# gasparian/CRNN-OCR-lite

Measured on AMD Instinct MI355X. Metric: text-line images/sec (train step), higher is better.
Workload: dtype bf16; 1 GPU; BASELINE configs[1]: 100x32x1 text lines, batch 256/GPU, max_len 23, time_dense_size 128, n_units 256 BiLSTM, STN on, dropout on, CTC, Adam(1e-4,b1=.5,clipnorm 5), bf16 MFMA products, bf16 conv-stack tensors in HBM, fp32 accumulate/statistics/RNN/optimizer (outside the 1e-3 parity tolerance: see parity_mode for the fp32 step); global_batch=256, parallelism=dp1, parity_mode_backward_planes=2 (16 significant bits per factor; CRNN_FLAG_THREE_PLANE_BACKWARD = strict)

## Files before the change

### crnn-ocr-lite_amd/crnn_mi355x/native.py

```python
import ctypes
import os
import re
import subprocess

HERE = os.path.dirname(os.path.abspath(__file__))
PKG_ROOT = os.path.dirname(HERE)
REPO_ROOT = os.path.dirname(PKG_ROOT)
HEADER = os.path.join(REPO_ROOT, "include", "crnn_mi355x.h")
CSRC = os.path.join(PKG_ROOT, "csrc")
LIB_PATH = os.path.join(PKG_ROOT, "libcrnn_mi355x.so")
HOOKS_HEADER = os.path.join(REPO_ROOT, "include", "crnn_testhooks.h")
HOOKS_PATH = os.path.join(PKG_ROOT, "libcrnn_testhooks.so")
SOURCES = ["gemm.hip", "gemm_nt.hip", "gemm_wres.hip", "gemm_wres3.hip", "gemm_wgrad.hip", "gemm_wgrad3.hip", "gemm_pres.hip", "conv.hip", "conv_bwd_fused.hip", "dwconv_stream.hip", "dwconv_bwd_stream.hip", "stn.hip", "rnn.hip", "rnn_persist.hip", "gru_persist.hip", "ctc.hip", "dense.hip", "beam.hip", "score.hip", "optim.hip", "ingest.hip", "model.hip"]


class crnn_config(ctypes.Structure):
    _fields_ = [(n, ctypes.c_int) for n in
                ("batch", "imgh", "imgw", "num_classes", "max_len", "tds", "units", "gru", "stn", "dropout", "mfma_bf16", "flags")]


FLAG_RNN_STEP_KERNELS = 1
FLAG_GEMM_TILE_KERNELS = 2
FLAG_NO_DW_BN_FUSION = 8
FLAG_NO_DW_BWD_FUSION = 16
FLAG_DW_TILE_KERNEL = 32
FLAG_RNN_LINEAR_CLUSTERS = 64
FLAG_NO_BN_STATS_FUSION = 128
FLAG_F32_MFMA_GEMMS = 256
FLAG_BN2_DW_FUSION = 1024
FLAG_BN2_STATS_FUSION = 2048
FLAG_BLOCK1_KERNELS = 16384
FLAG_LOC_NET_KERNELS = 8192
FLAG_THREE_PLANE_BACKWARD = 65536
FLAG_TWO_PLANE_FORWARD = 131072
FLAG_NO_GRADIENT_PLANES = 262144
FLAG_NO_POOL_ARGMAX_Q = 524288
FLAG_NO_BN2_DW_FUSION = 4096
RNN_XCD_LOCAL = 0x100


_CTYPE = [("crnn_stream_t", ctypes.c_void_p), ("size_t", ctypes.c_size_t), ("uint64_t", ctypes.c_uint64),
          ("uint32_t", ctypes.c_uint32), ("long", ctypes.c_long), ("int", ctypes.c_int), ("float", ctypes.c_float),
          ("double", ctypes.c_double)]


def _ctype_of(decl):
    decl = decl.strip()
    if "*" in decl:
        return ctypes.c_void_p
    for key, ct in _CTYPE:
        if re.search(r"\b%s\b" % key, decl):
            return ct
    raise ValueError("cannot map C type: %r" % decl)


def parse_header(path=HEADER):
    src = open(path).read()
    src = re.sub(r"/\*.*?\*/", " ", src, flags=re.S)
    src = re.sub(r"typedef\s+struct\s*\{.*?\}\s*\w+\s*;", " ", src, flags=re.S)
# ... 83 lines not shown
```

### crnn-ocr-lite_amd/csrc/conv.hip

```cpp
#include "common.h"
#include <stdlib.h>

#define BN_EPS 1e-3f
#ifndef DW_NT
#define DW_NT 256
#endif

template <int VEC>
struct VecF { float v[VEC]; };

#ifndef CRNN_NT_BN_BWD2
#define CRNN_NT_BN_BWD2 1
#endif
#ifndef CRNN_NT_BN_ACT
#define CRNN_NT_BN_ACT 1
#endif
template <int VEC, typename T>
__device__ __forceinline__ VecF<VEC> vload_nt(const T* p);
template <int VEC, bool NT, typename T>
__device__ __forceinline__ VecF<VEC> vload_s(const T* p);
template <int VEC, typename T>
__device__ __forceinline__ VecF<VEC> vload(const T* p) {
  VecF<VEC> r;
  if (VEC == 8) {
// ... 1508 lines not shown
    for (int r = rt; r < 128 && r0 + r < M; r += RT) {
      const float av = relu6f(fmaf(d[r0 + r], sc, sh));
      VecF<8> o;
#pragma unroll
      for (int e = 0; e < 8; ++e) o.v[e] = av * wv[e];
      vstore<8>(&q[(r0 + r) * N + 8 * cg], o);
#pragma unroll
      for (int e = 0; e < 8; ++e) {
        float v = o.v[e];
        if (sizeof(T) == 2) v = __uint_as_float(pack2_bf16(v, 0.f) << 16);
        s[e] += v; ss[e] = fmaf(v, v, ss[e]);
      }
    }
#pragma unroll
  for (int e = 0; e < 8; ++e) { red[0][tid * 8 + e] = s[e]; red[1][tid * 8 + e] = ss[e]; }
  __syncthreads();
  if (tid < 2 * N) {
    const int v = tid / N, c = tid % N;
    float acc = 0.f;
    for (int r = 0; r < RT; ++r) acc += red[v][(r * CG + c / 8) * 8 + (c & 7)];
    stats[((long)blockIdx.x * 2 + v) * N + c] = acc;
  }
}
template <typename T>
__global__ __launch_bounds__(256) void pw1_bn_bwd_kernel(const float* __restrict__ d, const float* __restrict__ bn1, const float* __restrict__ w,
                                                         const T* __restrict__ dq, float* __restrict__ da, float* __restrict__ partials,
                                                         float* __restrict__ bnparts, long M, int N, int rows_per_chunk) {
  __shared__ float red[256 * 8];
  __shared__ float sred[2][256];
  const int CG = N / 8, RT = 256 / CG, tid = threadIdx.x, cg = tid % CG, rt = tid / CG;
  const long r0 = (long)blockIdx.x * rows_per_chunk;
  long r1 = r0 + rows_per_chunk; if (r1 > M) r1 = M;
  const float mu = bn1[0], inv = 1.0f / sqrtf(bn1[1] + BN_EPS), sc = bn1[2], sh = bn1[3];
  VecF<8> wl = vload<8>(w + 8 * cg);
  float s[8], sg = 0.f, sq = 0.f;
#pragma unroll
  for (int e = 0; e < 8; ++e) s[e] = 0.f;
  if (rt < RT)
    for (long r = r0 + rt; r < r1; r += RT) {
      const float dv = d[r], t = fmaf(dv, sc, sh), av = relu6f(t);
      VecF<8> g = vload<8>(&dq[r * N + 8 * cg]);
      float acc = 0.f;
#pragma unroll
      for (int e = 0; e < 8; ++e) { s[e] = fmaf(av, g.v[e], s[e]); acc = fmaf(g.v[e], wl.v[e], acc); }
      for (int o = 1; o < CG; o <<= 1) acc += __shfl_xor(acc, o, 64);
      if (cg == 0) {
        da[r] = acc;
        const float gy = (t > 0.f && t < 6.f) ? acc : 0.f;
        sg += gy; sq = fmaf(gy, (dv - mu) * inv, sq);
      }
    }
#pragma unroll
  for (int e = 0; e < 8; ++e) red[tid * 8 + e] = s[e];
  sred[0][tid] = sg; sred[1][tid] = sq;
  __syncthreads();
  if (tid < N) {
    float acc = 0.f;
    for (int r = 0; r < RT; ++r) acc += red[(r * CG + tid / 8) * 8 + (tid & 7)];
    partials[(long)blockIdx.x * N + tid] = acc;
  }
  if (tid < 2) {
    float acc = 0.f;
    for (int r = 0; r < RT; ++r) acc += sred[tid][r * CG];
    bnparts[(long)blockIdx.x * 2 + tid] = acc;
// ... 141 lines not shown
  if (!pw1_ok(N, q) || M <= 0) return CRNN_ERR_UNSUPPORTED;
  const int blocks = cdiv(M, 128);
  if (dt_q == CRNN_BF16) hipLaunchKernelGGL(pw1_bn_fwd_kernel<bf16_t>, dim3(blocks), dim3(256), 0, stream, d, in_bnstate, w, (bf16_t*)q, stat_partials, M, N);
  else hipLaunchKernelGGL(pw1_bn_fwd_kernel<float>, dim3(blocks), dim3(256), 0, stream, d, in_bnstate, w, (float*)q, stat_partials, M, N);
  CRNN_LAUNCH_CHECK();
  return CRNN_OK;
}
extern "C" int crnn_dwconv_c1_bwd_rows(int B, int H, int W) { return cdiv((long)B * H * W, 1024); }
extern "C" int crnn_dwconv3x3_c1_bwd(const float* d, const float* da, const float* bnstate, const float* coef, const float* x, const float* k, float* dx, float* dk,
                                     float* scratch, int B, int H, int W, hipStream_t stream) {
  if (!d || !da || !bnstate || !coef || !x || !k || !dk || !scratch || B <= 0 || H <= 0 || W <= 0) return CRNN_ERR_ARG;
  if ((long)B * H * W >= (1L << 31) || W > C1B_MAXW) return CRNN_ERR_UNSUPPORTED;
  const int rows = crnn_dwconv_c1_bwd_rows(B, H, W);
  hipLaunchKernelGGL(dwconv_c1_bwd_kernel, dim3(rows), dim3(256), 0, stream, d, da, bnstate, coef, x, k, dx, scratch, B, H, W);
  CRNN_LAUNCH_CHECK();
  return crnn_partials_sum(scratch, rows, 9, dk, 1.f, stream);
}
extern "C" int crnn_pw1_bn_bwd_rows(long M) { return cdiv(M, colreduce_rpc(M)); }
extern "C" int crnn_pw1_bn_bwd(const float* d, const float* in_bnstate, const float* w, const void* dq, float* da, float* dw, float* scratch,
                               float* bn_stat_partials, long M, int N, int dt_q, hipStream_t stream) {
  if (!d || !in_bnstate || !w || !dq || !da || !dw || !scratch || !bn_stat_partials) return CRNN_ERR_ARG;
  if (!pw1_ok(N, dq) || M <= 0 || N < 8) return CRNN_ERR_UNSUPPORTED;
  const int rpc = colreduce_rpc(M), chunks = cdiv(M, rpc);
  if (dt_q == CRNN_BF16) hipLaunchKernelGGL(pw1_bn_bwd_kernel<bf16_t>, dim3(chunks), dim3(256), 0, stream, d, in_bnstate, w, (const bf16_t*)dq, da, scratch, bn_stat_partials, M, N, rpc);
  else hipLaunchKernelGGL(pw1_bn_bwd_kernel<float>, dim3(chunks), dim3(256), 0, stream, d, in_bnstate, w, (const float*)dq, da, scratch, bn_stat_partials, M, N, rpc);
  CRNN_LAUNCH_CHECK();
  return crnn_partials_sum(scratch, chunks, N, dw, 1.f, stream);
}
```

### crnn-ocr-lite_amd/csrc/model.hip

```cpp
#include "common.h"
#include "crnn_mi355x.h"
#include <string.h>
#include <stdio.h>
#include <string>
#include <vector>

namespace {

struct BlockSpec { int cout, ph, pw; };
const BlockSpec kBlocks[7] = {{64, 1, 1}, {128, 1, 1}, {256, 2, 2}, {256, 1, 1}, {512, 1, 2}, {512, 1, 1}, {512, 1, 1}};
bool pool_argmax_q(const crnn_config* cfg, int block) {
  const int ph = kBlocks[block - 1].ph, pw = kBlocks[block - 1].pw;
  return !(cfg->flags & CRNN_FLAG_NO_POOL_ARGMAX_Q) && ((ph == 2 && pw == 2) || (ph == 1 && pw == 2));
}
const float kDropBlock = 0.1f, kDropDense1 = 0.4f, kDropRnn = 0.2f;
const uint32_t kLayerDense1 = 8, kLayerRnn = 9;

struct Tensor { std::string name; long off; long size; int ndim; int dims[4]; int dtype = CRNN_F32; };

struct Dims {
  int B, H0, W0, Hp, Wp, T, feat, C, L, tds, u, G, stn_flat;
  int Hs1, Ws1, Ho1, Wo1, Hs2, Ws2, Ho2, Wo2;
  int bh[8], bw[8], bc[8];
};
// ... 939 lines not shown
  Ctx ca = c; if (aux) { ca.s = aux; ca.side = true; }
  float* gA = c.w("gA"); float* gB = c.w("gB"); float* gC = c.w("gC");
  hipEvent_t gB_free = nullptr, gC_free = nullptr;
  int bn2_stats_rows = 0;
  for (int i = 7; i >= 1; --i) {
    std::string p = std::to_string(i), bp = "b" + p;
    const int H = d.bh[i], W = d.bw[i], ci = d.bc[i - 1], co = d.bc[i];
    const long M = (long)B * H * W;
    const int dtd = c.dt("d" + p), dtq = c.dt("q" + p);
    const bool fused_bf = i > 1 && dtd == CRNN_BF16 && c.dt("x" + std::to_string(i - 1)) == CRNN_BF16 && !(cfg->flags & CRNN_FLAG_NO_DW_BWD_FUSION) &&
                          crnn_dwconv_bwd_fused_supported(H, W, ci) == CRNN_OK;
    const bool fused_f32 = i > 1 && dtd == CRNN_F32 && dtq == CRNN_F32 && c.dt("x" + std::to_string(i - 1)) == CRNN_F32 &&
                           !(cfg->flags & (CRNN_FLAG_NO_DW_BWD_FUSION | CRNN_FLAG_DW_TILE_KERNEL)) &&
                           crnn_dwconv_bwd_stream_supported_ex(B, H, W, ci, CRNN_F32) == CRNN_OK &&
                           aligned16(c.w("d" + p), c.w("x" + std::to_string(i - 1)), c.p(bp + "_dw"), c.w("coef")) && aligned16(gA, gB, gC, c.w("bn1s" + p));
    const bool fused_dw = fused_bf || fused_f32;
    int bn1_stats_rows = 0;
    const bool dq_planes = !fused_bf && pw_products(cfg) == 2 && conv_planes(cfg, true) == 2 && dtq == CRNN_F32 && dtd == CRNN_F32 && fuse_dw_bn_x3(cfg, dtd, dtq, ci) &&
                           !(cfg->flags & (CRNN_FLAG_GEMM_TILE_KERNELS | CRNN_FLAG_NO_BN_STATS_FUSION | CRNN_FLAG_NO_GRADIENT_PLANES)) &&
                           (kBlocks[i - 1].ph * kBlocks[i - 1].pw == 1 || crnn_knob("CRNN_DQPL_POOL", 1)) &&
                           crnn_gemm_pres_supported(M, ci, co, 2) == CRNN_OK && crnn_pwconv_wgrad_planes_stream_supported(M, co, ci) == CRNN_OK &&
                           crnn_pwconv_wgrad_planes_stream_scratch_bytes(M, co, ci) <= kGemmScratchBytes &&
                           aligned16(c.w("d" + p), c.w("q" + p), c.w("bn1s" + p), c.p(bp + "_pw")) && aligned16(gA, gB, gC, c.w("partials"));
    CRNN_TRY(fj.wait(gB_free)); gB_free = nullptr;
    if (bn2_stats_rows > 0) {
      CRNN_TRY(crnn_bn_bwd_finalize(c.w("bn2parts"), bn2_stats_rows, co, M, c.g(bp + "_bn2_g"), c.g(bp + "_bn2_b"), c.w("coef"), stream));
      if (dq_planes)
        CRNN_TRY(crnn_bn_bwd_apply_planes_ex(c.w("q" + p), gA, c.w("bn2s" + p), c.w("coef"), gB, M * co, 2, B, H, W, co, kBlocks[i - 1].ph, kBlocks[i - 1].pw,
                                             cfg->dropout ? kDropBlock : 0.f, seed, (uint32_t)i, stream));
      else
      CRNN_TRY(crnn_bn_bwd_apply_ex(c.w("q" + p), gA, c.w("bn2s" + p), c.w("coef"), gB, B, H, W, co, kBlocks[i - 1].ph, kBlocks[i - 1].pw,
                                    cfg->dropout ? kDropBlock : 0.f, seed, (uint32_t)i, dtq, stream));
      bn2_stats_rows = 0;
    } else if (use_qmax(c, i))
      CRNN_TRY(crnn_bn_bwd_qmax_ex(c.w("q" + p), c.w("qm" + p), gA, c.w("bn2s" + p), c.p(bp + "_bn2_g"), dq_planes ? nullptr : gB, dq_planes ? gB : nullptr, M * co,
                                   dq_planes ? 2 : 0, c.g(bp + "_bn2_g"), c.g(bp + "_bn2_b"), c.w("partials"), c.w("coef"), B, H, W, co, kBlocks[i - 1].ph,
                                   kBlocks[i - 1].pw, cfg->dropout ? kDropBlock : 0.f, seed, (uint32_t)i, dtq, stream));
    else if (dq_planes)
      CRNN_TRY(crnn_bn_bwd_planes_ex(c.w("q" + p), gA, c.w("bn2s" + p), c.p(bp + "_bn2_g"), gB, M * co, 2, c.g(bp + "_bn2_g"), c.g(bp + "_bn2_b"), c.w("partials"),
                                     c.w("coef"), B, H, W, co, kBlocks[i - 1].ph, kBlocks[i - 1].pw, cfg->dropout ? kDropBlock : 0.f, seed, (uint32_t)i, stream));
    else
    CRNN_TRY(crnn_bn_bwd_ex(c.w("q" + p), gA, c.w("bn2s" + p), c.p(bp + "_bn2_g"), gB, c.g(bp + "_bn2_g"), c.g(bp + "_bn2_b"), c.w("partials"),
                            c.w("coef"), B, H, W, co, kBlocks[i - 1].ph, kBlocks[i - 1].pw, cfg->dropout ? kDropBlock : 0.f, seed, (uint32_t)i, dtq, stream));
    if (block1_fused(cfg, ci, dtd)) {
      const int rows = crnn_pw1_bn_bwd_rows(M);
      float* bnp = c.w("partials");
      CRNN_TRY(crnn_pw1_bn_bwd(c.w("d" + p), c.w("bn1s" + p), c.p(bp + "_pw"), gB, gA, c.g(bp + "_pw"), bnp + ((2L * rows + 63) & ~63L), bnp, M, co, dtq, stream));
      bn1_stats_rows = rows;
    } else if (ci == 1 && dtd == CRNN_F32) {
      CRNN_TRY(crnn_pw1_bwd(c.w("a" + p), c.p(bp + "_pw"), gB, gA, c.g(bp + "_pw"), c.w("partials"), M, co, dtq, stream));
    } else {
      const bool side = fj.on && fused_dw;
      const Ctx& cw = side ? ca : c;
      if (side) CRNN_TRY(fj.fork());
      if (fuse_dw_bn(cfg, dtd, dtq, ci)) {
        int rc = CRNN_ERR_UNSUPPORTED;
        if (!(cfg->flags & CRNN_FLAG_GEMM_TILE_KERNELS) && crnn_pwconv_wgrad_stream_supported(M, co, ci) == CRNN_OK)
          rc = crnn_pwconv_bnrelu6_wgrad_stream(c.w("d" + p), c.w("bn1s" + p), gB, c.g(bp + "_pw"), M, co, ci, cw.scratch(), kGemmScratchBytes, cw.s);
        if (rc == CRNN_ERR_UNSUPPORTED)
          rc = crnn_pwconv_bnrelu6_wgrad(c.w("d" + p), c.w("bn1s" + p), gB, c.g(bp + "_pw"), M, co, ci, cw.scratch(), kGemmScratchBytes, cw.s);
        CRNN_TRY(rc);
      }
      else if (fuse_dw_bn_x3(cfg, dtd, dtq, ci) && aligned16(c.w("d" + p), c.w("q" + p), c.w("bn1s" + p), c.p(bp + "_pw"))) {
        int rc = CRNN_ERR_UNSUPPORTED;
        if (dq_planes) { CRNN_TRY(crnn_pwconv_bnrelu6_wgrad_planes_stream_gp(c.w("d" + p), c.w("bn1s" + p), gB, M * co, c.g(bp + "_pw"), M, co, ci, cw.scratch(), kGemmScratchBytes, cw.s)); rc = CRNN_OK; }
        if (rc == CRNN_ERR_UNSUPPORTED)
          rc = (conv_planes(cfg, true) == 2 ? crnn_pwconv_bnrelu6_wgrad_f32x2 : crnn_pwconv_bnrelu6_wgrad_f32x3)(
              c.w("d" + p), c.w("bn1s" + p), gB, c.g(bp + "_pw"), M, co, ci, cw.scratch(), kGemmScratchBytes, cw.s);
        CRNN_TRY(rc);
      }
      else CRNN_TRY(gemm_t(cw, 2, c.w("a" + p), dtd, gB, dtq, c.g(bp + "_pw"), CRNN_F32, ci, co, (int)M, ci, co, co, nullptr, 0, 0, 0, conv_planes(cfg, true)));
// ... 148 lines not shown
```

### include/crnn_mi355x.h

```cpp
#ifndef CRNN_MI355X_H
#define CRNN_MI355X_H
#include <stddef.h>
#include <stdint.h>
#ifdef __cplusplus
extern "C" {
#endif

typedef struct ihipStream_t* crnn_stream_t;

typedef struct {
  int batch;
  int imgh, imgw;
  int num_classes;
  int max_len;
  int tds;
  int units;
  int gru;
  int stn;
  int dropout;
  int mfma_bf16;
  int flags;
} crnn_config;
#define CRNN_FLAG_BLOCK1_KERNELS 16384
#define CRNN_FLAG_LOC_NET_KERNELS 8192
#define CRNN_FLAG_NO_BN2_DW_FUSION 4096
#define CRNN_FLAG_BN2_STATS_FUSION 2048
#define CRNN_FLAG_BN2_DW_FUSION 1024
#define CRNN_FLAG_DW_TILE_KERNEL 32
#define CRNN_FLAG_NO_DW_BWD_FUSION 16
#define CRNN_FLAG_NO_DW_BN_FUSION 8
#define CRNN_FLAG_GEMM_TILE_KERNELS 2
#define CRNN_FLAG_THREE_PLANE_BACKWARD 65536
#define CRNN_FLAG_TWO_PLANE_FORWARD 131072
#define CRNN_FLAG_NO_GRADIENT_PLANES 262144
#define CRNN_FLAG_NO_POOL_ARGMAX_Q 524288
#define CRNN_FLAG_F32_MFMA_GEMMS 256
#define CRNN_FLAG_NO_BN_STATS_FUSION 128
#define CRNN_FLAG_RNN_LINEAR_CLUSTERS 64
#define CRNN_FLAG_RNN_STEP_KERNELS 1

int  crnn_num_params(const crnn_config* cfg);
long crnn_params_total(const crnn_config* cfg);
int  crnn_param_info(const crnn_config* cfg, int idx, char* name, int name_cap, long* offset, long* size,
                     int* ndim, int* dims );
int  crnn_bn_total(const crnn_config* cfg);
int  crnn_bn_info(const crnn_config* cfg, int idx, char* name, int name_cap, int* offset, int* channels, long* count);
int  crnn_time_steps(const crnn_config* cfg);

size_t crnn_workspace_bytes(const crnn_config* cfg);
int  crnn_ws_tensor(const crnn_config* cfg, const char* name, long* offset, long* count);
int  crnn_block_output_fused(const crnn_config* cfg, int block);
int  crnn_ws_tensor_info(const crnn_config* cfg, const char* name, long* offset, long* count, int* dtype);


int crnn_forward(const crnn_config* cfg, const float* params, const float* bn_mean, const float* bn_var,
                 const float* x, float* ws, size_t ws_bytes, float* y_pred, int train, uint64_t seed,
                 crnn_stream_t stream);
int crnn_forward_ex(const crnn_config* cfg, const float* params, const float* bn_mean, const float* bn_var,
// ... 85 lines not shown
int crnn_pwconv_bnrelu6_wgrad_planes_stream_gp(const float* d, const float* in_bnstate, const void* g_planes, long g_plane_stride, float* dw, long M, int N, int K,
                                               float* scratch, size_t scratch_bytes, crnn_stream_t stream);
int crnn_gemm_tn_planes_stream(const float* A, int lda, const float* B, int ldb, float* C, int ldc, int M, int N, long K, float* scratch,
                               size_t scratch_bytes, crnn_stream_t stream);
int crnn_gemm_nt_f32x2_stream(const float* A0, const float* W0, const float* A1, const float* W1, float* Y, int M, int N, int K, int lda, int ldw, int ldy,
                              crnn_stream_t stream);
int crnn_gemm_pres_supported(long M, int N, int K, int planes);
int crnn_gemm_pres_stat_rows(long M, int N, int K, int planes);
int crnn_gemm_pres_bnstats(const void* dq_planes, long plane_stride, const float* w, float* da, long M, int N, int K, int planes, const float* d,
                           const float* bnstate, float* stat_partials, void* a_planes, long a_stride, int a_count, crnn_stream_t stream);
int crnn_pw1_fwd(const float* a, const float* w, void* q, long M, int N, float* stat_partials, int dt_q, crnn_stream_t stream);
int crnn_pw1_fwd_folded(const float* a, const float* w, void* y, long M, int N, const float* out_bnstate, int dt_y, crnn_stream_t stream);
int crnn_pw1_bwd(const float* a, const float* w, const void* dq, float* da, float* dw, float* scratch, long M, int N, int dt_q,
                 crnn_stream_t stream);
int crnn_dwconv_c1_stat_rows(int B, int H, int W);
int crnn_dwconv3x3_c1_fwd(const float* x, const float* k, float* out, float* stat_partials, int B, int H, int W, crnn_stream_t stream);
int crnn_pw1_bn_fwd(const float* d, const float* in_bnstate, const float* w, void* q, long M, int N, float* stat_partials, int dt_q, crnn_stream_t stream);
int crnn_dwconv_c1_bwd_rows(int B, int H, int W);
int crnn_dwconv3x3_c1_bwd(const float* d, const float* da, const float* bnstate, const float* coef, const float* x, const float* k, float* dx, float* dk,
                          float* scratch, int B, int H, int W, crnn_stream_t stream);
int crnn_pw1_bn_bwd_rows(long M);
int crnn_pw1_bn_bwd(const float* d, const float* in_bnstate, const float* w, const void* dq, float* da, float* dw, float* scratch, float* bn_stat_partials,
                    long M, int N, int dt_q, crnn_stream_t stream);
int crnn_dwconv3x3_bn_relu6_fwd(const void* x, const float* k, const float* bnstate, void* out, int B, int H, int W, int C,
                                int dtype, crnn_stream_t stream);
int crnn_dwconv_fwd_stream_supported(int B, int H, int W, int C);
int crnn_dwconv_fwd_stream_rows(int B, int H, int W, int C);
int crnn_dwconv3x3_fwd_stream(const void* x, const float* k, void* out, float* stat_partials, const float* bnstate, int B, int H, int W, int C,
                              int flip, crnn_stream_t stream);
int crnn_dwconv3x3_fwd_stream_ex(const void* x, const float* k, void* out, float* stat_partials, const float* bnstate, int B, int H, int W, int C,
                                 int flip, int out_order, crnn_stream_t stream);
int crnn_dwconv_fwd_stream_pro_supported(int B, int H, int W, int C);
int crnn_dwconv3x3_fwd_stream_pro(const void* q, const float* pro_bnstate, float rate, const void* keep, const float* k, void* out,
                                  float* stat_partials, int B, int H, int W, int C, crnn_stream_t stream);
int crnn_transpose_batch(const float* src, void* dst, int n, const long* in_off, const long* out_off, const int* R, const int* C,
                         int dt_out, crnn_stream_t stream);
int crnn_dwconv3x3_fwd_ex(const void* x, const float* k, void* out, float* stat_partials, int B, int H, int W, int C, int flip,
                          int dtype, crnn_stream_t stream);
int crnn_dwconv3x3_wgrad_ex(const void* x, const void* g, float* dk, float* scratch, int B, int H, int W, int C, int dtype,
                            crnn_stream_t stream);
int crnn_colreduce_ex(const void* x, float* partials, long M, int C, int ld, int nv, int dtype, crnn_stream_t stream);
int crnn_bn_act_pool_drop_ex(const void* x, const float* bnstate, void* y, int B, int H, int W, int C, int ph, int pw, float rate,
                             uint64_t seed, uint32_t layer, int dt_in, int dt_out, crnn_stream_t stream);
int crnn_bn_bwd_ex(const void* x, const void* g, const float* bnstate, const float* gamma, void* dx, float* dgamma, float* dbeta,
                   float* scratch_partials, float* coef, int B, int H, int W, int C, int ph, int pw, float rate, uint64_t seed,
                   uint32_t layer, int dtype, crnn_stream_t stream);
// ... 213 lines not shown
```

Baseline: 43560 images/sec.

## Fuse BN2 backward apply into pointwise-conv backward kernels to skip dq materialization

Adds a fused pointwise-conv backward kernel (MFMA bf16) that recomputes the BN2/ReLU6/dropout backward input gradient on the fly from q and g. It also computes the BN1-relu6 activation from d and produces both da and the weight gradient in one pass. A variant of the block-1 pw1 backward kernel applies the BN backward inline the same way. This removes the separate bn_bwd apply pass and the HBM round trip of the dq tensor for unpooled blocks. It adds a large, complex kernel with split-K partial reductions and more launch conditions.

```diff
diff --git a/crnn-ocr-lite_amd/crnn_mi355x/native.py b/crnn-ocr-lite_amd/crnn_mi355x/native.py
--- a/crnn-ocr-lite_amd/crnn_mi355x/native.py
+++ b/crnn-ocr-lite_amd/crnn_mi355x/native.py
@@ -11,7 +11,7 @@
 LIB_PATH = os.path.join(PKG_ROOT, "libcrnn_mi355x.so")
 HOOKS_HEADER = os.path.join(REPO_ROOT, "include", "crnn_testhooks.h")
 HOOKS_PATH = os.path.join(PKG_ROOT, "libcrnn_testhooks.so")
-SOURCES = ["gemm.hip", "gemm_nt.hip", "gemm_wres.hip", "gemm_wres3.hip", "gemm_wgrad.hip", "gemm_wgrad3.hip", "gemm_pres.hip", "conv.hip", "conv_bwd_fused.hip", "dwconv_stream.hip", "dwconv_bwd_stream.hip", "stn.hip", "rnn.hip", "rnn_persist.hip", "gru_persist.hip", "ctc.hip", "dense.hip", "beam.hip", "score.hip", "optim.hip", "ingest.hip", "model.hip"]
+SOURCES = ["gemm.hip", "gemm_nt.hip", "gemm_wres.hip", "gemm_wres3.hip", "gemm_wgrad.hip", "gemm_wgrad3.hip", "gemm_pres.hip", "gemm_pwbwd.hip", "conv.hip", "conv_bwd_fused.hip", "dwconv_stream.hip", "dwconv_bwd_stream.hip", "stn.hip", "rnn.hip", "rnn_persist.hip", "gru_persist.hip", "ctc.hip", "dense.hip", "beam.hip", "score.hip", "optim.hip", "ingest.hip", "model.hip"]
 
 
 class crnn_config(ctypes.Structure):
@@ -35,6 +35,7 @@
 FLAG_TWO_PLANE_FORWARD = 131072
 FLAG_NO_GRADIENT_PLANES = 262144
 FLAG_NO_POOL_ARGMAX_Q = 524288
+FLAG_NO_PW_BWD_FUSION = 1048576
 FLAG_NO_BN2_DW_FUSION = 4096
 RNN_XCD_LOCAL = 0x100
 
diff --git a/crnn-ocr-lite_amd/csrc/conv.hip b/crnn-ocr-lite_amd/csrc/conv.hip
--- a/crnn-ocr-lite_amd/csrc/conv.hip
+++ b/crnn-ocr-lite_amd/csrc/conv.hip
@@ -1554,10 +1554,11 @@
     stats[((long)blockIdx.x * 2 + v) * N + c] = acc;
   }
 }
-template <typename T>
+template <typename T, bool APPLY = false>
 __global__ __launch_bounds__(256) void pw1_bn_bwd_kernel(const float* __restrict__ d, const float* __restrict__ bn1, const float* __restrict__ w,
                                                          const T* __restrict__ dq, float* __restrict__ da, float* __restrict__ partials,
-                                                         float* __restrict__ bnparts, long M, int N, int rows_per_chunk) {
+                                                         float* __restrict__ bnparts, long M, int N, int rows_per_chunk, BnBwdArgsT<T> ap,
+                                                         const float* __restrict__ coef) {
   __shared__ float red[256 * 8];
   __shared__ float sred[2][256];
   const int CG = N / 8, RT = 256 / CG, tid = threadIdx.x, cg = tid % CG, rt = tid / CG;
@@ -1568,10 +1569,36 @@
   float s[8], sg = 0.f, sq = 0.f;
 #pragma unroll
   for (int e = 0; e < 8; ++e) s[e] = 0.f;
+  VecF<8> sc2, sh2, Pc, Qc;
+  float inv_keep = 1.f;
+  if constexpr (APPLY) {
+    const int c0 = 8 * cg;
+    const VecF<8> mu2 = vload<8>(ap.bnstate + c0), var2 = vload<8>(ap.bnstate + N + c0);
+    sc2 = vload<8>(ap.bnstate + 2 * N + c0); sh2 = vload<8>(ap.bnstate + 3 * N + c0);
+    const VecF<8> c1 = vload<8>(coef + c0), c2 = vload<8>(coef + N + c0);
+#pragma unroll
+    for (int e = 0; e < 8; ++e) bn_bwd_pq(sc2.v[e], c1.v[e], c2.v[e], mu2.v[e], 1.0f / sqrtf(var2.v[e] + BN_EPS), Pc.v[e], Qc.v[e]);
+    inv_keep = ap.rate > 0.f ? 1.f / (1.f - ap.rate) : 1.f;
+  }
   if (rt < RT)
     for (long r = r0 + rt; r < r1; r += RT) {
       const float dv = d[r], t = fmaf(dv, sc, sh), av = relu6f(t);
-      VecF<8> g = vload<8>(&dq[r * N + 8 * cg]);
+      VecF<8> g;
+      if constexpr (APPLY) {
+        const VecF<8> xv = vload<8>(&ap.x[r * N + 8 * cg]);
+        const VecF<8> gy = bn_gy_vec<8, false, T>(ap, r, 8 * cg, xv, sc2, sh2, inv_keep);
+#pragma unroll
+        for (int e = 0; e < 8; ++e) g.v[e] = bn_bwd_dx_pq(xv.v[e], gy.v[e], sc2.v[e], Pc.v[e], Qc.v[e]);
+        if constexpr (sizeof(T) == 2) {
+#pragma unroll
+          for (int e = 0; e < 8; e += 2) {
+            const unsigned pk = pack2_bf16(g.v[e], g.v[e + 1]);
+            g.v[e] = __uint_as_float(pk << 16); g.v[e + 1] = __uint_as_float(pk & 0xffff0000u);
+          }
+        }
+      } else {
+        g = vload<8>(&dq[r * N + 8 * cg]);
+      }
       float acc = 0.f;
 #pragma unroll
       for (int e = 0; e < 8; ++e) { s[e] = fmaf(av, g.v[e], s[e]); acc = fmaf(g.v[e], wl.v[e], acc); }
@@ -1759,8 +1786,29 @@
   if (!d || !in_bnstate || !w || !dq || !da || !dw || !scratch || !bn_stat_partials) return CRNN_ERR_ARG;
   if (!pw1_ok(N, dq) || M <= 0 || N < 8) return CRNN_ERR_UNSUPPORTED;
   const int rpc = colreduce_rpc(M), chunks = cdiv(M, rpc);
-  if (dt_q == CRNN_BF16) hipLaunchKernelGGL(pw1_bn_bwd_kernel<bf16_t>, dim3(chunks), dim3(256), 0, stream, d, in_bnstate, w, (const bf16_t*)dq, da, scratch, bn_stat_partials, M, N, rpc);
-  else hipLaunchKernelGGL(pw1_bn_bwd_kernel<float>, dim3(chunks), dim3(256), 0, stream, d, in_bnstate, w, (const float*)dq, da, scratch, bn_stat_partials, M, N, rpc);
+  if (dt_q == CRNN_BF16) hipLaunchKernelGGL(pw1_bn_bwd_kernel<bf16_t>, dim3(chunks), dim3(256), 0, stream, d, in_bnstate, w, (const bf16_t*)dq, da, scratch, bn_stat_partials, M, N, rpc, BnBwdArgsT<bf16_t>{}, nullptr);
+  else hipLaunchKernelGGL(pw1_bn_bwd_kernel<float>, dim3(chunks), dim3(256), 0, stream, d, in_bnstate, w, (const float*)dq, da, scratch, bn_stat_partials, M, N, rpc, BnBwdArgsT<float>{}, nullptr);
   CRNN_LAUNCH_CHECK();
   return crnn_partials_sum(scratch, chunks, N, dw, 1.f, stream);
 }
+template <typename T>
+static void pw1_apply_launch(const float* d, const float* in_bnstate, const float* w, const void* q, const void* g, const float* out_bnstate, const float* coef,
+                             float rate, uint64_t seed, uint32_t layer, float* da, float* scratch, float* bn_stat_partials, long M, int N, int rpc, int chunks,
+                             hipStream_t stream) {
+  BnBwdArgsT<T> ap{};
+  ap.x = (const T*)q; ap.g = (const T*)g; ap.bnstate = out_bnstate; ap.gamma = nullptr;
+  ap.B = 1; ap.H = 1; ap.W = 1; ap.C = N; ap.ph = 1; ap.pw = 1; ap.rate = rate; ap.seed = seed; ap.layer = layer;
+  hipLaunchKernelGGL((pw1_bn_bwd_kernel<T, true>), dim3(chunks), dim3(256), 0, stream, d, in_bnstate, w, (const T*)nullptr, da, scratch, bn_stat_partials, M, N, rpc, ap, coef);
+}
+extern "C" int crnn_pw1_bn_bwd_apply(const float* d, const float* in_bnstate, const float* w, const void* q, const void* g, const float* out_bnstate,
+                                     const float* coef, float rate, uint64_t seed, uint32_t layer, float* da, float* dw, float* scratch,
+                                     float* bn_stat_partials, long M, int N, int dt_q, hipStream_t stream) {
+  if (!d || !in_bnstate || !w || !q || !g || !out_bnstate || !coef || !da || !dw || !scratch || !bn_stat_partials) return CRNN_ERR_ARG;
+  if (!pw1_ok(N, q) || M <= 0 || N < 8) return CRNN_ERR_UNSUPPORTED;
+  if ((((uintptr_t)g | (uintptr_t)out_bnstate | (uintptr_t)coef) & 15)) return CRNN_ERR_UNSUPPORTED;
+  const int rpc = colreduce_rpc(M), chunks = cdiv(M, rpc);
+  if (dt_q == CRNN_BF16) pw1_apply_launch<bf16_t>(d, in_bnstate, w, q, g, out_bnstate, coef, rate, seed, layer, da, scratch, bn_stat_partials, M, N, rpc, chunks, stream);
+  else pw1_apply_launch<float>(d, in_bnstate, w, q, g, out_bnstate, coef, rate, seed, layer, da, scratch, bn_stat_partials, M, N, rpc, chunks, stream);
+  CRNN_LAUNCH_CHECK();
+  return crnn_partials_sum(scratch, chunks, N, dw, 1.f, stream);
+}
diff --git a/crnn-ocr-lite_amd/csrc/gemm_pwbwd.hip b/crnn-ocr-lite_amd/csrc/gemm_pwbwd.hip
--- /dev/null
+++ b/crnn-ocr-lite_amd/csrc/gemm_pwbwd.hip
@@ -0,0 +1,361 @@
+#include "common.h"
+
+typedef __bf16 bf16x8_t __attribute__((ext_vector_type(8)));
+typedef unsigned u32x2 __attribute__((ext_vector_type(2)));
+typedef unsigned u32x4 __attribute__((ext_vector_type(4)));
+typedef short s16x4 __attribute__((ext_vector_type(4)));
+
+#ifndef CRNN_PWB_EXP
+#define CRNN_PWB_EXP 0
+#endif
+
+namespace {
+
+struct PwbParams {
+  const bf16_t* Q; const bf16_t* G; const bf16_t* D; const bf16_t* W; bf16_t* DA;
+  const float* bn2; const float* coef; const float* bn1;
+  float* part; float* stats;
+  long M; int stripes;
+  int unit, nunits;
+  float rate; uint64_t seed; uint32_t layer;
+};
+
+constexpr int kLdQ = 320, kLdA = 192, kLdO = 128;
+
+__device__ __forceinline__ unsigned pwb_bnrelu6_pair(unsigned w, float s0, float s1, float t0, float t1) {
+  f32x2_t v;
+  v[0] = fma_unpacked(__uint_as_float(w << 16), s0, t0);
+  v[1] = fma_unpacked(__uint_as_float(w & 0xffff0000u), s1, t1);
+  v[0] = __builtin_amdgcn_fmed3f(v[0], 0.f, 6.f); v[1] = __builtin_amdgcn_fmed3f(v[1], 0.f, 6.f);
+  return __builtin_bit_cast(unsigned, __builtin_convertvector(v, bf16x2_t));
+}
+template <int LD, bool SW>
+__device__ __forceinline__ bf16x8_t pwb_frag_tr(const unsigned char* Xs, int r0, int ks, int half, int l31) {
+  const int li = l31 & 15;
+  const int row = ks * 16 + 8 * half + (li >> 2), col = r0 + (l31 & 16) + (li & 3) * 4;
+  const int ch = col >> 3, sw0 = SW ? (row >> 2) & 3 : 0, sw1 = SW ? ((row + 4) >> 2) & 3 : 0;
+  const unsigned char* X0 = Xs + row * LD + (((ch & ~3) | ((ch & 3) ^ sw0)) << 4) + (col & 7) * 2;
+  const unsigned char* X1 = Xs + (row + 4) * LD + (((ch & ~3) | ((ch & 3) ^ sw1)) << 4) + (col & 7) * 2;
+  const s16x4 lo = __builtin_amdgcn_ds_read_tr16_b64_v4i16((__attribute__((address_space(3))) s16x4*)X0);
+  const s16x4 hi = __builtin_amdgcn_ds_read_tr16_b64_v4i16((__attribute__((address_space(3))) s16x4*)X1);
+  const uint2 a = __builtin_bit_cast(uint2, lo), b = __builtin_bit_cast(uint2, hi);
+  return __builtin_bit_cast(bf16x8_t, make_uint4(a.x, a.y, b.x, b.y));
+}
+__device__ __forceinline__ void pwb_sync() {
+  asm volatile("s_waitcnt lgkmcnt(0)" ::: "memory");
+  __builtin_amdgcn_s_barrier();
+}
+
+template <int CI, int CO, bool STATS>
+__global__ __launch_bounds__(512) void pw_bwd_fused_kernel(PwbParams p) {
+  static_assert(CI == 64 && CO == 128, "thread maps: 16 q pieces x 32 rows, 8 d pieces x 64 rows, 8 waves = 2 x 4 MFMA blocks for either product");
+  constexpr int KS = CO / 16;
+  constexpr int oA = 128 * kLdQ, oO = oA + 128 * kLdA, oT = oO + 128 * kLdO, oW = oT + (4 * CO + 4 * CI) * (int)sizeof(float);
+  extern __shared__ __attribute__((aligned(16))) unsigned char smem[];
+  unsigned char* const dqs = smem;
+  unsigned char* const as = smem + oA;
+  unsigned char* const outs = smem + oO;
+  unsigned char* const wls = smem + oW;
+  float* const tab2_ = reinterpret_cast<float*>(smem + oT);
+  float* const tab1_ = tab2_ + 4 * CO;
+  const int tid = threadIdx.x, lane = tid & 63;
+  const int wave = __builtin_amdgcn_readfirstlane(tid >> 6);
+  const int half = lane >> 5, l31 = lane & 31;
+  const int wg = blockIdx.x, nwg = gridDim.x;
+  const int u0 = (int)((long)wg * p.nunits / nwg), u1 = (int)((long)(wg + 1) * p.nunits / nwg);
+  const int s0 = u0 * p.unit, s1 = min(u1 * p.unit, p.stripes);
+
+  for (int i = tid; i < CO; i += 512) {
+    const float mu = p.bn2[i], inv = 1.0f / sqrtf(p.bn2[CO + i] + 1e-3f), sc = p.bn2[2 * CO + i];
+    float P, Q;
+    bn_bwd_pq(sc, p.coef[i], p.coef[CO + i], mu, inv, P, Q);
+    tab2_[i] = sc; tab2_[CO + i] = p.bn2[3 * CO + i]; tab2_[2 * CO + i] = P; tab2_[3 * CO + i] = Q;
+  }
+  for (int i = tid; i < CI; i += 512) {
+    tab1_[i] = p.bn1[2 * CI + i]; tab1_[CI + i] = p.bn1[3 * CI + i];
+    tab1_[2 * CI + i] = p.bn1[i]; tab1_[3 * CI + i] = 1.0f / sqrtf(p.bn1[CI + i] + 1e-3f);
+  }
+  const int cb = wave & 1, pb = wave >> 1;
+  if (wave < CI / 32) {
+    const bf16_t* wrow = p.W + (long)(32 * wave + l31) * CO + half * 8;
+#pragma unroll
+    for (int ks = 0; ks < KS; ++ks) *reinterpret_cast<u32x4*>(wls + ((wave * KS + ks) * 64 + lane) * 16) = *reinterpret_cast<const u32x4*>(wrow + ks * 16);
+  }
+  const f32x16 zero16 = {0.f, 0.f, 0.f, 0.f, 0.f, 0.f, 0.f, 0.f, 0.f, 0.f, 0.f, 0.f, 0.f, 0.f, 0.f, 0.f};
+  f32x16 accw = zero16;
+  const float inv_keep = p.rate > 0.f ? 1.f / (1.f - p.rate) : 1.f;
+
+  const int qc = tid & 15, qr = tid >> 4;
+  const int dc = tid & 7, dr = tid >> 3;
+  u32x4 rq[4], rg[4], rd[2];
+  auto load = [&](int s) {
+    const long base = (long)s * 128;
+#pragma unroll
+    for (int u = 0; u < 4; ++u) {
+      long row = base + qr + 32 * u; row = row < p.M ? row : p.M - 1;
+      if (CRNN_PWB_EXP & 4) { rq[u] = u32x4{(unsigned)s, 0u, 0u, 0u}; rg[u] = rq[u]; continue; }
+      rq[u] = *reinterpret_cast<const u32x4*>(p.Q + row * CO + qc * 8);
+      rg[u] = *reinterpret_cast<const u32x4*>(p.G + row * CO + qc * 8);
+    }
+#pragma unroll
+    for (int u = 0; u < 2; ++u) {
+      long row = base + dr + 64 * u; row = row < p.M ? row : p.M - 1;
+      if (CRNN_PWB_EXP & 4) { rd[u] = u32x4{(unsigned)s, 0u, 0u, 0u}; continue; }
+      rd[u] = *reinterpret_cast<const u32x4*>(p.D + row * CI + dc * 8);
+    }
+  };
+  float ss[8], qq[8];
+#pragma unroll
+  for (int e = 0; e < 8; ++e) { ss[e] = 0.f; qq[e] = 0.f; }
+
+  load(s0);
+  __syncthreads();
+  for (int s = s0; s < s1; ++s) {
+    const long base = (long)s * 128;
+    u32x4 dcur[2];
+    int tz = 0;
+    asm volatile("" : "+v"(tz));
+    const float* const tab2 = tab2_ + tz;
+    const float* const tab1 = tab1_ + tz;
+    {
+      float sc[8], sh[8], P[8], Q[8];
+#pragma unroll
+      for (int h = 0; h < 2; ++h) {
+        const float4 a0 = *reinterpret_cast<const float4*>(tab2 + qc * 8 + 4 * h), a1 = *reinterpret_cast<const float4*>(tab2 + CO + qc * 8 + 4 * h);
+        const float4 a2 = *reinterpret_cast<const float4*>(tab2 + 2 * CO + qc * 8 + 4 * h), a3 = *reinterpret_cast<const float4*>(tab2 + 3 * CO + qc * 8 + 4 * h);
+        sc[4 * h] = a0.x; sc[4 * h + 1] = a0.y; sc[4 * h + 2] = a0.z; sc[4 * h + 3] = a0.w;
+        sh[4 * h] = a1.x; sh[4 * h + 1] = a1.y; sh[4 * h + 2] = a1.z; sh[4 * h + 3] = a1.w;
+        P[4 * h] = a2.x; P[4 * h + 1] = a2.y; P[4 * h + 2] = a2.z; P[4 * h + 3] = a2.w;
+        Q[4 * h] = a3.x; Q[4 * h + 1] = a3.y; Q[4 * h + 2] = a3.z; Q[4 * h + 3] = a3.w;
+      }
+#pragma unroll
+      for (int u = 0; u < 4; ++u) {
+        const int lr = qr + 32 * u;
+        const long row = base + lr;
+        u32x4 o;
+        if (CRNN_PWB_EXP & 1) o = rq[u] ^ rg[u]; else {
+        float dm[8];
+        drop_scale_vec<8>(p.seed, p.layer, (uint64_t)(row * CO + qc * 8), p.rate, inv_keep, dm);
+        const unsigned xw[4] = {rq[u].x, rq[u].y, rq[u].z, rq[u].w}, gw[4] = {rg[u].x, rg[u].y, rg[u].z, rg[u].w};
+        unsigned ow[4];
+#pragma unroll
+        for (int w = 0; w < 4; ++w) {
+          float r2[2];
+#pragma unroll
+          for (int hf = 0; hf < 2; ++hf) {
+            const int e = 2 * w + hf;
+            const float x = __uint_as_float(hf ? (xw[w] & 0xffff0000u) : (xw[w] << 16));
+            const float gv = __uint_as_float(hf ? (gw[w] & 0xffff0000u) : (gw[w] << 16));
+            const float t = fmaf(x, sc[e], sh[e]);
+            const bool live = (t > 0.f) && (t < 6.f);
+            const float gy = live ? gv * dm[e] : 0.f;
+            r2[hf] = bn_bwd_dx_pq(x, gy, sc[e], P[e], Q[e]);
+          }
+          ow[w] = pack2_bf16(r2[0], r2[1]);
+        }
+        o = u32x4{ow[0], ow[1], ow[2], ow[3]};
+        }
+        if (row >= p.M) o = u32x4{0u, 0u, 0u, 0u};
+        *reinterpret_cast<u32x4*>(dqs + lr * kLdQ + (((qc & ~3) | ((qc & 3) ^ ((lr >> 2) & 3))) << 4)) = o;
+        __builtin_amdgcn_sched_barrier(0);
+      }
+      const float4 s0v = *reinterpret_cast<const float4*>(tab1 + dc * 8), s1v = *reinterpret_cast<const float4*>(tab1 + dc * 8 + 4);
+      const float4 t0v = *reinterpret_cast<const float4*>(tab1 + CI + dc * 8), t1v = *reinterpret_cast<const float4*>(tab1 + CI + dc * 8 + 4);
+#pragma unroll
+      for (int u = 0; u < 2; ++u) {
+        const int lr = dr + 64 * u;
+        u32x4 o;
+        if (CRNN_PWB_EXP & 1) o = rd[u]; else {
+        o.x = pwb_bnrelu6_pair(rd[u].x, s0v.x, s0v.y, t0v.x, t0v.y);
+        o.y = pwb_bnrelu6_pair(rd[u].y, s0v.z, s0v.w, t0v.z, t0v.w);
+        o.z = pwb_bnrelu6_pair(rd[u].z, s1v.x, s1v.y, t1v.x, t1v.y);
+        o.w = pwb_bnrelu6_pair(rd[u].w, s1v.z, s1v.w, t1v.z, t1v.w);
+        }
+        if (base + lr >= p.M) o = u32x4{0u, 0u, 0u, 0u};
+        *reinterpret_cast<u32x4*>(as + lr * kLdA + dc * 16) = o;
+        if (STATS) dcur[u] = rd[u];
+      }
+    }
+    __builtin_amdgcn_sched_barrier(0);
+    if (s + 1 < s1) load(s + 1);
+    pwb_sync();
+    if (!(CRNN_PWB_EXP & 2)) {
+      f32x16 acc;
+      const int px = 32 * pb + l31;
+      const unsigned char* xrow = dqs + px * kLdQ;
+      const int sw = (px >> 2) & 3;
+#pragma unroll
+      for (int ks = 0; ks < KS; ++ks) {
+        const int ch = 2 * ks + half;
+        const bf16x8_t fx = *reinterpret_cast<const bf16x8_t*>(xrow + (((ch & ~3) | ((ch & 3) ^ sw)) << 4));
+        const bf16x8_t wf = *reinterpret_cast<const bf16x8_t*>(wls + ((cb * KS + ks) * 64 + lane) * 16);
+        acc = __builtin_amdgcn_mfma_f32_32x32x16_bf16(wf, fx, ks == 0 ? zero16 : acc, 0, 0, 0);
+      }
+#pragma unroll
+      for (int pr = 0; pr < 2; ++pr) {
+        unsigned g0a = pack2_bf16(acc[8 * pr + 0], acc[8 * pr + 1]), g0b = pack2_bf16(acc[8 * pr + 2], acc[8 * pr + 3]);
+        unsigned g1a = pack2_bf16(acc[8 * pr + 4], acc[8 * pr + 5]), g1b = pack2_bf16(acc[8 * pr + 6], acc[8 * pr + 7]);
+        const u32x2 sa = __builtin_amdgcn_permlane32_swap(g0a, g1a, false, false);
+        const u32x2 sb = __builtin_amdgcn_permlane32_swap(g0b, g1b, false, false);
+        *reinterpret_cast<uint4*>(outs + px * kLdO + (((4 * cb + 2 * pr + half) ^ ((px >> 1) & 7)) << 4)) = make_uint4(sa.x, sb.x, sa.y, sb.y);
+      }
+#pragma unroll
+      for (int ks = 0; ks < 8; ++ks) {
+        const bf16x8_t fa = pwb_frag_tr<kLdA, false>(as, 32 * cb, ks, half, l31);
+        const bf16x8_t fb = pwb_frag_tr<kLdQ, true>(dqs, 32 * pb, ks, half, l31);
+        accw = __builtin_amdgcn_mfma_f32_32x32x16_bf16(fa, fb, accw, 0, 0, 0);
+      }
+    }
+    __builtin_amdgcn_sched_barrier(0);
+    if ((s + 1) % p.unit == 0 || s + 1 == s1) {
+      float* out = p.part + (long)(s / p.unit) * CI * CO;
+#pragma unroll
+      for (int e = 0; e < 16; ++e) out[(32 * cb + 8 * (e >> 2) + 4 * half + (e & 3)) * CO + 32 * pb + l31] = accw[e];
+      accw = zero16;
+    }
+    pwb_sync();
+    {
+      const float4 s0v = *reinterpret_cast<const float4*>(tab1 + dc * 8), s1v = *reinterpret_cast<const float4*>(tab1 + dc * 8 + 4);
+      const float4 t0v = *reinterpret_cast<const float4*>(tab1 + CI + dc * 8), t1v = *reinterpret_cast<const float4*>(tab1 + CI + dc * 8 + 4);
+      const float4 m0v = *reinterpret_cast<const float4*>(tab1 + 2 * CI + dc * 8), m1v = *reinterpret_cast<const float4*>(tab1 + 2 * CI + dc * 8 + 4);
+      const float4 i0v = *reinterpret_cast<const float4*>(tab1 + 3 * CI + dc * 8), i1v = *reinterpret_cast<const float4*>(tab1 + 3 * CI + dc * 8 + 4);
+      const float sc[8] = {s0v.x, s0v.y, s0v.z, s0v.w, s1v.x, s1v.y, s1v.z, s1v.w}, sh[8] = {t0v.x, t0v.y, t0v.z, t0v.w, t1v.x, t1v.y, t1v.z, t1v.w};
+      const float mu[8] = {m0v.x, m0v.y, m0v.z, m0v.w, m1v.x, m1v.y, m1v.z, m1v.w}, inv[8] = {i0v.x, i0v.y, i0v.z, i0v.w, i1v.x, i1v.y, i1v.z, i1v.w};
+#pragma unroll
+      for (int u = 0; u < 2; ++u) {
+        const int lr = dr + 64 * u;
+        const long row = base + lr;
+        const u32x4 v = *reinterpret_cast<const u32x4*>(outs + lr * kLdO + ((dc ^ ((lr >> 1) & 7)) << 4));
+        if (row < p.M) *reinterpret_cast<u32x4*>(p.DA + row * CI + dc * 8) = v;
+        if (STATS && row < p.M) {
+#pragma clang fp contract(off)
+          const unsigned gw[4] = {v.x, v.y, v.z, v.w}, xw[4] = {dcur[u].x, dcur[u].y, dcur[u].z, dcur[u].w};
+#pragma unroll
+          for (int w = 0; w < 4; ++w)
+#pragma unroll
+            for (int hf = 0; hf < 2; ++hf) {
+              const int e = 2 * w + hf;
+              const float xx = __uint_as_float(hf ? (xw[w] & 0xffff0000u) : (xw[w] << 16));
+              const float gg = __uint_as_float(hf ? (gw[w] & 0xffff0000u) : (gw[w] << 16));
+              const float t = fmaf(xx, sc[e], sh[e]);
+              const float gy = (t > 0.f && t < 6.f) ? gg : 0.f;
+              const float xh = (xx - mu[e]) * inv[e];
+              ss[e] += gy;
+              qq[e] = fmaf(gy, xh, qq[e]);
+            }
+        }
+        __builtin_amdgcn_sched_barrier(0);
+      }
+    }
+  }
+  if (!STATS) return;
+  float* red = reinterpret_cast<float*>(dqs);
+#pragma unroll
+  for (int e = 0; e < 8; ++e) {
+    ss[e] += __shfl_xor(ss[e], 8, 64); qq[e] += __shfl_xor(qq[e], 8, 64);
+    ss[e] += __shfl_xor(ss[e], 16, 64); qq[e] += __shfl_xor(qq[e], 16, 64);
+    ss[e] += __shfl_xor(ss[e], 32, 64); qq[e] += __shfl_xor(qq[e], 32, 64);
+  }
+  if (lane < 8) {
+#pragma unroll
+    for (int e = 0; e < 8; ++e) { red[(wave * 2 + 0) * CI + lane * 8 + e] = ss[e]; red[(wave * 2 + 1) * CI + lane * 8 + e] = qq[e]; }
+  }
+  __syncthreads();
+  if (tid < 2 * CI) {
+    float acc = 0.f;
+    for (int w = 0; w < 8; ++w) acc += red[w * 2 * CI + tid];
+    p.stats[(long)wg * 2 * CI + tid] = acc;
+  }
+}
+
+constexpr int kPwbLds = 128 * (kLdQ + kLdA + kLdO) + (4 * 128 + 4 * 64) * (int)sizeof(float) + 64 * 128 * 2;
+
+template <int LY>
+__global__ __launch_bounds__(32 * LY) void pwb_range_sum_kernel(const float* __restrict__ part, int nsplit, int nreal, long total, float* __restrict__ out) {
+  __shared__ float red[LY][33];
+  const long i = (long)blockIdx.x * 32 + threadIdx.x;
+  auto at = [&](int z) { return z < nreal ? part[(long)z * total + i] : 0.f; };
+  float s = 0.f;
+  if (i < total) {
+    int z = threadIdx.y;
+    for (; z + 3 * LY < nsplit; z += 4 * LY) {
+      const float v0 = at(z), v1 = at(z + LY), v2 = at(z + 2 * LY), v3 = at(z + 3 * LY);
+      s += (v0 + v1) + (v2 + v3);
+    }
+    for (; z < nsplit; z += LY) s += at(z);
+  }
+  red[threadIdx.y][threadIdx.x] = s;
+  __syncthreads();
+  if (threadIdx.y == 0 && i < total) {
+    s = 0.f;
+#pragma unroll
+    for (int r = 0; r < LY; r += 4) s += (red[r][threadIdx.x] + red[r + 1][threadIdx.x]) + (red[r + 2][threadIdx.x] + red[r + 3][threadIdx.x]);
+    out[i] = s;
+  }
+}
+__global__ __launch_bounds__(256) void pwb_range_sum8_kernel(const float* __restrict__ part, int nreal, long total, float* __restrict__ out) {
+  const long i = (long)blockIdx.x * 256 + threadIdx.x;
+  if (i >= total) return;
+  float a[8];
+#pragma unroll
+  for (int z = 0; z < 8; ++z) a[z] = z < nreal ? part[(long)z * total + i] : 0.f;
+  out[i] = ((a[0] + a[1]) + (a[2] + a[3])) + ((a[4] + a[5]) + (a[6] + a[7]));
+}
+
+struct PwbGeom { int unit, nunits, nsplit, grid; };
+PwbGeom pwb_geom(long M, int max_workgroups = 0) {
+  const long K = M;
+  long nsplit = 1;
+  if (K >= 512) { nsplit = 768; const long maxs = K / (K >= 2048 ? 512 : 128); if (nsplit > maxs) nsplit = maxs; if (nsplit < 1) nsplit = 1; }
+  long klen = (K + nsplit - 1) / nsplit; klen = (klen + 63) / 64 * 64;
+  nsplit = (K + klen - 1) / klen;
+  if (nsplit >= 8) { const long ns8 = (nsplit + 7) / 8 * 8; klen = (K + ns8 - 1) / ns8; klen = (klen + 63) / 64 * 64; nsplit = ns8; }
+  if (klen % 128) { klen = (klen + 127) / 128 * 128; nsplit = (K + klen - 1) / klen; }
+  PwbGeom g;
+  g.unit = (int)(klen / 128); g.nunits = (int)((K + klen - 1) / klen); g.nsplit = (int)nsplit;
+  int dev = 0, cus = 0;
+  if (hipGetDevice(&dev) != hipSuccess || hipDeviceGetAttribute(&cus, hipDeviceAttributeMultiprocessorCount, dev) != hipSuccess || cus < 1) cus = 256;
+  g.grid = g.nunits < cus ? g.nunits : cus;
+  if (max_workgroups > 0 && g.grid > max_workgroups) g.grid = max_workgroups;
+  return g;
+}
+
+}
+
+extern "C" int crnn_pwconv_bwd_fused_supported(long M, int ci, int co) {
+  return (M > 0 && M < (1L << 31) && ci == 64 && co == 128) ? CRNN_OK : CRNN_ERR_UNSUPPORTED;
+}
+extern "C" int crnn_pwconv_bwd_fused_stat_rows(long M, int ci, int co) {
+  return crnn_pwconv_bwd_fused_supported(M, ci, co) == CRNN_OK ? pwb_geom(M).grid : 0;
+}
+extern "C" size_t crnn_pwconv_bwd_fused_scratch_bytes(long M, int ci, int co) {
+  return crnn_pwconv_bwd_fused_supported(M, ci, co) == CRNN_OK ? (size_t)pwb_geom(M).nunits * ci * co * sizeof(float) : 0;
+}
+extern "C" int crnn_pwconv_bwd_fused(const void* q, const void* g, const float* out_bnstate, const float* coef, float rate, uint64_t seed, uint32_t layer,
+                                     const void* d, const float* in_bnstate, const void* w_bf16, void* da, float* dw, float* scratch, size_t scratch_bytes,
+                                     float* stat_partials, long stat_partials_floats, long M, int ci, int co, int max_workgroups, hipStream_t stream) {
+  if (!q || !g || !out_bnstate || !coef || !d || !in_bnstate || !w_bf16 || !da || !dw || !scratch) return CRNN_ERR_ARG;
+  CRNN_TRY(crnn_pwconv_bwd_fused_supported(M, ci, co));
+  if ((((uintptr_t)q | (uintptr_t)g | (uintptr_t)out_bnstate | (uintptr_t)coef | (uintptr_t)d | (uintptr_t)in_bnstate | (uintptr_t)w_bf16 | (uintptr_t)da |
+        (uintptr_t)dw | (uintptr_t)scratch | (uintptr_t)stat_partials) & 15)) return CRNN_ERR_UNSUPPORTED;
+  const PwbGeom gm = pwb_geom(M, max_workgroups);
+  if ((size_t)gm.nunits * ci * co * sizeof(float) > scratch_bytes || (stat_partials && (long)gm.grid * 2 * ci > stat_partials_floats)) return CRNN_ERR_UNSUPPORTED;
+  PwbParams p;
+  p.Q = (const bf16_t*)q; p.G = (const bf16_t*)g; p.D = (const bf16_t*)d; p.W = (const bf16_t*)w_bf16; p.DA = (bf16_t*)da;
+  p.bn2 = out_bnstate; p.coef = coef; p.bn1 = in_bnstate; p.part = scratch; p.stats = stat_partials;
+  p.M = M; p.stripes = (int)((M + 127) / 128); p.unit = gm.unit; p.nunits = gm.nunits; p.rate = rate; p.seed = seed; p.layer = layer;
+  if (stat_partials) {
+    CRNN_LDS_ATTR((pw_bwd_fused_kernel<64, 128, true>), kPwbLds);
+    hipLaunchKernelGGL((pw_bwd_fused_kernel<64, 128, true>), dim3(gm.grid), dim3(512), kPwbLds, stream, p);
+  } else {
+    CRNN_LDS_ATTR((pw_bwd_fused_kernel<64, 128, false>), kPwbLds);
+    hipLaunchKernelGGL((pw_bwd_fused_kernel<64, 128, false>), dim3(gm.grid), dim3(512), kPwbLds, stream, p);
+  }
+  CRNN_LAUNCH_CHECK();
+  const long total = (long)ci * co;
+  if (gm.nsplit <= 8) hipLaunchKernelGGL(pwb_range_sum8_kernel, dim3(cdiv(total, 256)), dim3(256), 0, stream, scratch, gm.nunits, total, dw);
+  else if (gm.nsplit > 32) hipLaunchKernelGGL(pwb_range_sum_kernel<32>, dim3(cdiv(total, 32)), dim3(32, 32), 0, stream, scratch, gm.nsplit, gm.nunits, total, dw);
+  else hipLaunchKernelGGL(pwb_range_sum_kernel<8>, dim3(cdiv(total, 32)), dim3(32, 8), 0, stream, scratch, gm.nsplit, gm.nunits, total, dw);
+  CRNN_LAUNCH_CHECK();
+  return CRNN_OK;
+}
diff --git a/crnn-ocr-lite_amd/csrc/model.hip b/crnn-ocr-lite_amd/csrc/model.hip
--- a/crnn-ocr-lite_amd/csrc/model.hip
+++ b/crnn-ocr-lite_amd/csrc/model.hip
@@ -985,8 +985,23 @@
                            crnn_gemm_pres_supported(M, ci, co, 2) == CRNN_OK && crnn_pwconv_wgrad_planes_stream_supported(M, co, ci) == CRNN_OK &&
                            crnn_pwconv_wgrad_planes_stream_scratch_bytes(M, co, ci) <= kGemmScratchBytes &&
                            aligned16(c.w("d" + p), c.w("q" + p), c.w("bn1s" + p), c.p(bp + "_pw")) && aligned16(gA, gB, gC, c.w("partials"));
+    const bool unpooled = kBlocks[i - 1].ph * kBlocks[i - 1].pw == 1;
+    const bool pw1_apply = block1_fused(cfg, ci, dtd) && dtq == CRNN_BF16 && unpooled && !(cfg->flags & CRNN_FLAG_NO_PW_BWD_FUSION) &&
+                           aligned16(c.w("q" + p), gA, c.w("bn2s" + p), c.w("coef"));
+    int dtw2 = CRNN_F32;
+    const float* wsh2 = weight_operand(c, 1, c.p(bp + "_pw"), &dtw2);
+    const bool pw_fused = i > 1 && fused_dw && unpooled && fuse_dw_bn(cfg, dtd, dtq, ci) && dtw2 == CRNN_BF16 &&
+                          !(cfg->flags & (CRNN_FLAG_GEMM_TILE_KERNELS | CRNN_FLAG_NO_BN_STATS_FUSION | CRNN_FLAG_NO_DW_BN_FUSION | CRNN_FLAG_NO_DW_BWD_FUSION |
+                                          CRNN_FLAG_NO_PW_BWD_FUSION)) &&
+                          crnn_pwconv_bwd_fused_supported(M, ci, co) == CRNN_OK && crnn_pwconv_bwd_fused_scratch_bytes(M, ci, co) <= kGemmScratchBytes &&
+                          aligned16(c.w("q" + p), gA, gB, c.w("d" + p)) && aligned16(c.w("bn2s" + p), c.w("coef"), c.w("bn1s" + p), wsh2) &&
+                          aligned16(c.g(bp + "_pw"), c.scratch());
+    const bool no_dq = pw1_apply || pw_fused;
     CRNN_TRY(fj.wait(gB_free)); gB_free = nullptr;
-    if (bn2_stats_rows > 0) {
+    if (bn2_stats_rows > 0 && no_dq) {
+      CRNN_TRY(crnn_bn_bwd_finalize(c.w("bn2parts"), bn2_stats_rows, co, M, c.g(bp + "_bn2_g"), c.g(bp + "_bn2_b"), c.w("coef"), stream));
+      bn2_stats_rows = 0;
+    } else if (bn2_stats_rows > 0) {
       CRNN_TRY(crnn_bn_bwd_finalize(c.w("bn2parts"), bn2_stats_rows, co, M, c.g(bp + "_bn2_g"), c.g(bp + "_bn2_b"), c.w("coef"), stream));
       if (dq_planes)
         CRNN_TRY(crnn_bn_bwd_apply_planes_ex(c.w("q" + p), gA, c.w("bn2s" + p), c.w("coef"), gB, M * co, 2, B, H, W, co, kBlocks[i - 1].ph, kBlocks[i - 1].pw,
@@ -1003,13 +1018,24 @@
       CRNN_TRY(crnn_bn_bwd_planes_ex(c.w("q" + p), gA, c.w("bn2s" + p), c.p(bp + "_bn2_g"), gB, M * co, 2, c.g(bp + "_bn2_g"), c.g(bp + "_bn2_b"), c.w("partials"),
                                      c.w("coef"), B, H, W, co, kBlocks[i - 1].ph, kBlocks[i - 1].pw, cfg->dropout ? kDropBlock : 0.f, seed, (uint32_t)i, stream));
     else
-    CRNN_TRY(crnn_bn_bwd_ex(c.w("q" + p), gA, c.w("bn2s" + p), c.p(bp + "_bn2_g"), gB, c.g(bp + "_bn2_g"), c.g(bp + "_bn2_b"), c.w("partials"),
+    CRNN_TRY(crnn_bn_bwd_ex(c.w("q" + p), gA, c.w("bn2s" + p), c.p(bp + "_bn2_g"), no_dq ? nullptr : gB, c.g(bp + "_bn2_g"), c.g(bp + "_bn2_b"), c.w("partials"),
                             c.w("coef"), B, H, W, co, kBlocks[i - 1].ph, kBlocks[i - 1].pw, cfg->dropout ? kDropBlock : 0.f, seed, (uint32_t)i, dtq, stream));
-    if (block1_fused(cfg, ci, dtd)) {
+    if (pw1_apply) {
+      const int rows = crnn_pw1_bn_bwd_rows(M);
+      float* bnp = c.w("partials");
+      CRNN_TRY(crnn_pw1_bn_bwd_apply(c.w("d" + p), c.w("bn1s" + p), c.p(bp + "_pw"), c.w("q" + p), gA, c.w("bn2s" + p), c.w("coef"), cfg->dropout ? kDropBlock : 0.f,
+                                     seed, (uint32_t)i, gB, c.g(bp + "_pw"), bnp + ((2L * rows + 63) & ~63L), bnp, M, co, dtq, stream));
+      bn1_stats_rows = rows;
+      float* t = gA; gA = gB; gB = t;
+    } else if (block1_fused(cfg, ci, dtd)) {
       const int rows = crnn_pw1_bn_bwd_rows(M);
       float* bnp = c.w("partials");
       CRNN_TRY(crnn_pw1_bn_bwd(c.w("d" + p), c.w("bn1s" + p), c.p(bp + "_pw"), gB, gA, c.g(bp + "_pw"), bnp + ((2L * rows + 63) & ~63L), bnp, M, co, dtq, stream));
       bn1_stats_rows = rows;
+    } else if (pw_fused) {
+      CRNN_TRY(crnn_pwconv_bwd_fused(c.w("q" + p), gA, c.w("bn2s" + p), c.w("coef"), cfg->dropout ? kDropBlock : 0.f, seed, (uint32_t)i, c.w("d" + p), c.w("bn1s" + p),
+                                     wsh2, gB, c.g(bp + "_pw"), c.scratch(), kGemmScratchBytes, nullptr, 0, M, ci, co, 0, stream));
+      float* t = gA; gA = gB; gB = t;
     } else if (ci == 1 && dtd == CRNN_F32) {
       CRNN_TRY(crnn_pw1_bwd(c.w("a" + p), c.p(bp + "_pw"), gB, gA, c.g(bp + "_pw"), c.w("partials"), M, co, dtq, stream));
     } else {
diff --git a/include/crnn_mi355x.h b/include/crnn_mi355x.h
--- a/include/crnn_mi355x.h
+++ b/include/crnn_mi355x.h
@@ -34,6 +34,7 @@
 #define CRNN_FLAG_TWO_PLANE_FORWARD 131072
 #define CRNN_FLAG_NO_GRADIENT_PLANES 262144
 #define CRNN_FLAG_NO_POOL_ARGMAX_Q 524288
+#define CRNN_FLAG_NO_PW_BWD_FUSION 1048576
 #define CRNN_FLAG_F32_MFMA_GEMMS 256
 #define CRNN_FLAG_NO_BN_STATS_FUSION 128
 #define CRNN_FLAG_RNN_LINEAR_CLUSTERS 64
@@ -165,6 +166,15 @@
 int crnn_pw1_bn_bwd_rows(long M);
 int crnn_pw1_bn_bwd(const float* d, const float* in_bnstate, const float* w, const void* dq, float* da, float* dw, float* scratch, float* bn_stat_partials,
                     long M, int N, int dt_q, crnn_stream_t stream);
+int crnn_pwconv_bwd_fused_supported(long M, int ci, int co);
+int crnn_pwconv_bwd_fused_stat_rows(long M, int ci, int co);
+size_t crnn_pwconv_bwd_fused_scratch_bytes(long M, int ci, int co);
+int crnn_pwconv_bwd_fused(const void* q, const void* g, const float* out_bnstate, const float* coef, float rate, uint64_t seed, uint32_t layer,
+                          const void* d, const float* in_bnstate, const void* w_bf16, void* da, float* dw, float* scratch, size_t scratch_bytes,
+                          float* stat_partials, long stat_partials_floats, long M, int ci, int co, int max_workgroups, crnn_stream_t stream);
+int crnn_pw1_bn_bwd_apply(const float* d, const float* in_bnstate, const float* w, const void* q, const void* g, const float* out_bnstate,
+                          const float* coef, float rate, uint64_t seed, uint32_t layer, float* da, float* dw, float* scratch,
+                          float* bn_stat_partials, long M, int N, int dt_q, crnn_stream_t stream);
 int crnn_dwconv3x3_bn_relu6_fwd(const void* x, const float* k, const float* bnstate, void* out, int B, int H, int W, int C,
                                 int dtype, crnn_stream_t stream);
 int crnn_dwconv_fwd_stream_supported(int B, int H, int W, int C);
```

After: 44570 images/sec, median of 6. 1.02x the previous value.
